# Patryk27/strolle

Measured on AMD Instinct MI355X. Metric: Mray/s (primary + shadow + GI rays traced per second, whole job), higher is better.
Workload: dtype f32

## Files before the change

include/strolle_hip.h:

```cpp
#ifndef STROLLE_HIP_H
#define STROLLE_HIP_H

#include <stddef.h>
#include <stdint.h>

#ifdef __cplusplus
extern "C" {
#endif

typedef struct StEngine StEngine;
typedef uint64_t StHandle;

enum StStatus {
    ST_OK = 0,
    ST_ERR_INVALID_ARGUMENT = 1,
    ST_ERR_NO_DEVICE = 2,
    ST_ERR_UNKNOWN_CAMERA = 3,
    ST_ERR_EMPTY_MESH = 4,
    ST_ERR_HIP = 5,
    ST_ERR_ATLAS_FULL = 6,
    ST_ERR_IO = 7,
    ST_ERR_PARSE = 8,
    ST_ERR_UNSUPPORTED = 9,
    ST_ERR_BVH_TOO_DEEP = 10,
// ... 303 lines not shown
    uint32_t alias_gi_history;
    uint32_t tile_map;
    uint32_t tile_map_denoise;
    int32_t side_priority;
    uint32_t staging;
    uint32_t double_buffer;
    uint32_t packed_base;
    uint32_t tick_timing;
    uint32_t anyhit_fast;
    uint32_t compact_bvh;
    uint32_t allow_deep_bvh;
    uint32_t device_bake;
    uint32_t wide_bvh;
    uint32_t wide_stack_entries;
    uint32_t primary_packets;
} StTuning;
int st_engine_get_tuning(StEngine* e, StTuning* out);
int st_engine_set_tuning(StEngine* e, const StTuning* tuning);

enum StArithmetic { ST_ARITH_FAST = 0, ST_ARITH_EXACT = 1 };
int st_engine_set_arithmetic(StEngine* e, int arithmetic);
int st_engine_get_arithmetic(StEngine* e, int* out);

enum StBufferId {
    ST_BUF_PRIM_GBUFFER_D0_A = 0, ST_BUF_PRIM_GBUFFER_D0_B = 1, ST_BUF_PRIM_GBUFFER_D1_A = 2, ST_BUF_PRIM_GBUFFER_D1_B = 3,
    ST_BUF_PRIM_SURFACE_MAP_A = 4, ST_BUF_PRIM_SURFACE_MAP_B = 5, ST_BUF_REPROJECTION_MAP = 6, ST_BUF_VELOCITY_MAP = 7,
    ST_BUF_DI_RESERVOIRS_0 = 8, ST_BUF_DI_RESERVOIRS_1 = 9, ST_BUF_DI_RESERVOIRS_2 = 10,
    ST_BUF_DI_DIFF_SAMPLES = 11, ST_BUF_DI_DIFF_PREV_COLORS = 12, ST_BUF_DI_DIFF_CURR_COLORS = 13,
    ST_BUF_DI_DIFF_MOMENTS_A = 14, ST_BUF_DI_DIFF_MOMENTS_B = 15, ST_BUF_DI_DIFF_STASH = 16, ST_BUF_DI_SPEC_SAMPLES = 17,
    ST_BUF_GI_D0 = 18, ST_BUF_GI_D1 = 19, ST_BUF_GI_D2 = 20,
    ST_BUF_GI_RESERVOIRS_0 = 21, ST_BUF_GI_RESERVOIRS_1 = 22, ST_BUF_GI_RESERVOIRS_2 = 23, ST_BUF_GI_RESERVOIRS_3 = 24,
    ST_BUF_GI_DIFF_SAMPLES = 25, ST_BUF_GI_DIFF_PREV_COLORS = 26, ST_BUF_GI_DIFF_CURR_COLORS = 27,
    ST_BUF_GI_DIFF_MOMENTS_A = 28, ST_BUF_GI_DIFF_MOMENTS_B = 29, ST_BUF_GI_DIFF_STASH = 30, ST_BUF_GI_SPEC_SAMPLES = 31,
// ... 75 lines not shown
```

rust/strolle-hip/src/ffi.rs:

```rust
#![allow(non_camel_case_types, dead_code)]
use std::ffi::c_void;
use std::os::raw::c_char;

#[repr(C)]
#[derive(Clone, Copy, Default)]
pub struct StMeshTriangle {
    pub positions: [[f32; 3]; 3],
    pub normals: [[f32; 3]; 3],
    pub uvs: [[f32; 2]; 3],
    pub tangents: [[f32; 4]; 3],
}

#[repr(C)]
#[derive(Clone, Copy, Default)]
pub struct StMaterial {
    pub base_color: [f32; 4],
    pub emissive: [f32; 4],
    pub perceptual_roughness: f32,
    pub metallic: f32,
    pub reflectance: f32,
    pub ior: f32,
    pub base_color_texture: u64,
    pub emissive_texture: u64,
    pub metallic_roughness_texture: u64,
// ... 28 lines not shown
    pub pos_x: u32,
    pub pos_y: u32,
    pub _pad: u32,
    pub transform: [f32; 16],
    pub projection: [f32; 16],
}

pub const ST_OK: i32 = 0;
pub const ST_FORMAT_RGBA32F: i32 = 0;
pub const ST_FORMAT_RGBA16F: i32 = 1;
pub const ST_FORMAT_RGBA8_UNORM_SRGB: i32 = 2;
pub const ST_FORMAT_BGRA8_UNORM_SRGB: i32 = 3;

pub const ST_ERR_BVH_TOO_DEEP: i32 = 10;
pub const ST_ERR_DIST: i32 = 11;

#[repr(C)]
#[derive(Clone, Copy, Default)]
pub struct StTuning {
    pub struct_size: u32,
    pub overlap: u32,
    pub fuse: u32,
    pub fuse_di_head: u32,
    pub fuse_spatial: u32,
    pub fuse_gi_sampling: u32,
    pub fuse_gi_validation: u32,
    pub fuse_gi_reprojection: u32,
    pub fuse_wavelet: u32,
    pub fuse_compose: u32,
    pub preview_both: u32,
// ... 4 lines not shown
    pub alias_gi_history: u32,
    pub tile_map: u32,
    pub tile_map_denoise: u32,
    pub side_priority: i32,
    pub staging: u32,
    pub double_buffer: u32,
    pub packed_base: u32,
    pub tick_timing: u32,
    pub anyhit_fast: u32,
    pub compact_bvh: u32,
    pub allow_deep_bvh: u32,
    pub device_bake: u32,
    pub wide_bvh: u32,
    pub wide_stack_entries: u32,
    pub primary_packets: u32,
}

#[repr(C)]
#[derive(Clone, Copy, PartialEq, Eq, Debug)]
pub struct StDistGrid {
    pub cols: u32,
    pub rows: u32,
    pub row_edge: [u32; 17],
    pub col_edge: [[u32; 17]; 16],
}

#[repr(C)]
#[derive(Clone, Copy, Default, PartialEq, Eq, Debug)]
pub struct StDistRect {
    pub x0: u32,
// ... 201 lines not shown
pub struct StDofDesc {
    pub struct_size: u32,
    pub flags: u32,
    pub samples: u32,
    pub focal_distance: f32,
    pub aperture_f_stops: f32,
    pub sensor_height: f32,
    pub max_radius: f32,
    pub focus_x: f32,
    pub focus_y: f32,
    pub _pad: u32,
}
extern "C" {
    pub fn st_camera_set_dof(e: *mut StEngine, camera: u64, desc: *const StDofDesc) -> i32;
    pub fn st_camera_get_dof(e: *mut StEngine, camera: u64, out: *mut StDofDesc, enabled: *mut i32) -> i32;
    pub fn st_dof_plan(desc: *const StDofDesc, width: u32, height: u32, samples: *mut u32, tiles_xy: *mut u32, taps_xyr: *mut f32) -> i32;
    pub fn st_dof_process(e: *mut StEngine, desc: *const StDofDesc, display: *const StDisplayDesc, projection: *const f32, color_device: *const c_void, depth_device: *const c_void, width: u32, height: u32, dst_device: *mut c_void, dst_format: i32, hip_stream: *mut c_void) -> i32;
}

pub type hipStream_t = *mut c_void;
extern "C" {
    pub fn hipMalloc(ptr: *mut *mut c_void, bytes: usize) -> i32;
    pub fn hipFree(ptr: *mut c_void) -> i32;
    pub fn hipHostMalloc(ptr: *mut *mut c_void, bytes: usize, flags: u32) -> i32;
    pub fn hipHostFree(ptr: *mut c_void) -> i32;
    pub fn hipStreamCreate(stream: *mut hipStream_t) -> i32;
    pub fn hipStreamDestroy(stream: hipStream_t) -> i32;
}
```

strolle_amd/api.py:

```python
from __future__ import annotations

import ctypes as C
import dataclasses
import enum
import math
import os
import sys
from typing import Optional, Sequence

import numpy as np

_HERE = os.path.dirname(os.path.abspath(__file__))
LIB_PATH = os.environ.get("STROLLE_HIP_LIB") or os.path.join(_HERE, "csrc", "libstrolle_hip.so")
if os.environ.get("STROLLE_HIP_LIB"):
    LIB_PATH = os.environ["STROLLE_HIP_LIB"]


class StMeshTriangle(C.Structure):
    _fields_ = [("positions", C.c_float * 9), ("normals", C.c_float * 9), ("uvs", C.c_float * 6), ("tangents", C.c_float * 12)]


class StSkinVertex(C.Structure):
    _fields_ = [("joints", C.c_uint16 * 4), ("weights", C.c_float * 4)]

# ... 44 lines not shown
    def describe(self):
        return {"cols": self.cols, "rows": self.rows, "row_edges": list(self.row_edge[:self.rows + 1]),
                "col_edges": [list(self.col_edge[k][:self.cols + 1]) for k in range(self.rows)]}


class StDistUniqueId(C.Structure):
    _fields_ = [("internal", C.c_char * 128)]


class StTuning(C.Structure):
    _fields_ = [(n, C.c_uint32) for n in ("struct_size", "overlap", "fuse", "fuse_di_head", "fuse_spatial", "fuse_gi_sampling", "fuse_gi_validation",
                                          "fuse_gi_reprojection", "fuse_wavelet", "fuse_compose", "preview_both", "variance_in_reproject",
                                          "lean_frame", "skip_scratch_stores", "di_head_on_main", "alias_gi_history", "tile_map", "tile_map_denoise")] + \
               [("side_priority", C.c_int32)] + \
               [(n, C.c_uint32) for n in ("staging", "double_buffer", "packed_base", "tick_timing", "anyhit_fast", "compact_bvh",
                                          "allow_deep_bvh", "device_bake", "wide_bvh", "wide_stack_entries", "primary_packets")]


PROFILE_MAX_KERNELS = 64


class StKernelProfile(C.Structure):
    _fields_ = [("name", C.c_char * 48), ("launches", C.c_uint32), ("total_ms", C.c_float), ("algorithmic_bytes", C.c_double), ("traversal_bytes", C.c_double)]


class StGltfOptions(C.Structure):
    _fields_ = [("first_handle", C.c_uint64), ("first_image_handle", C.c_uint64), ("override_mask", C.c_uint32), ("reflectance", C.c_float),
                ("perceptual_roughness", C.c_float), ("subdivide", C.c_uint32), ("light_radius", C.c_float), ("_pad", C.c_uint32)]


class StGltfSummary(C.Structure):
# ... 1183 lines not shown
```

strolle_amd/csrc/k_common.h:

```cpp
#pragma once
#include "st_device.h"
#include "st_passes.h"
#include "st_kernels.h"

namespace st {

constexpr int kBlockThreads = 256;
#ifdef ST_MIN_WAVES
#define ST_KERNEL_BOUNDS __launch_bounds__(kBlockThreads, ST_MIN_WAVES)
#else
#define ST_KERNEL_BOUNDS __launch_bounds__(kBlockThreads)
#endif
#define ST_STACK_LDS(SE, name) extern __shared__ __align__(16) unsigned char st_stack_lds_[]; SE* name = reinterpret_cast<SE*>(st_stack_lds_)
inline uint32_t stack_lds_bytes(const KArgs& a, size_t slot_bytes) { return a.stack_entries * (uint32_t)kBlockThreads * (uint32_t)slot_bytes; }

struct TileWindow { uint32_t tx0, tx1, ty0, ty1; };
__host__ __device__ inline TileWindow tile_window(const KArgs& a, bool half_x) {
    uint32_t tiles_x = (a.width + 7u) >> 3;
    if (half_x) tiles_x >>= 1;
    const uint32_t shift = half_x ? 4u : 3u, round = half_x ? 15u : 7u;
    TileWindow w;
    w.tx0 = a.col0 >> shift;
    w.tx1 = (a.col1 + round) >> shift; if (w.tx1 > tiles_x) w.tx1 = tiles_x;
    if (w.tx0 > w.tx1) w.tx0 = w.tx1;
// ... 2 lines not shown
    return w;
}
struct LaunchDims { uint32_t tiles_x, tile_x0, tile_y0, tile_y1, blocks; };
inline LaunchDims launch_dims(const KArgs& a, bool half_x) {
    const TileWindow w = tile_window(a, half_x);
    LaunchDims d;
    d.tiles_x = w.tx1 - w.tx0; d.tile_x0 = w.tx0;
    d.tile_y0 = w.ty0; d.tile_y1 = w.ty1;
    const uint32_t groups_x = (d.tiles_x + 3u) / 4u;
    d.blocks = groups_x * (d.tile_y1 - d.tile_y0);
    return d;
}

ST_D TileCoord resolve_tile(const KArgs& a, bool half_x) {
    const TileWindow w = tile_window(a, half_x);
    TileCoord tc = tile_for_thread(w.tx1 - w.tx0, w.ty1 - w.ty0, a.tile_map);
    tc.x += w.tx0; tc.y += w.ty0;
    return tc;
}
ST_D bool resolve_gid_of_block(const KArgs& a, bool half_x, uint32_t b, U2* gid) {
    const TileWindow w = tile_window(a, half_x);
    TileCoord tc = tile_for_block(b, w.tx1 - w.tx0, w.ty1 - w.ty0, a.tile_map);
    tc.x += w.tx0; tc.y += w.ty0;
    if (!tc.valid) return false;
    *gid = pixel_in_tile(tc);
    return true;
}
ST_D bool resolve_gid(const KArgs& a, bool half_x, U2* gid) {
    const TileCoord tc = resolve_tile(a, half_x);
    if (!tc.valid) return false;
    *gid = pixel_in_tile(tc);
    return true;
}
ST_D bool owns_pixel(const KArgs& a, U2 p) { return p.x < a.width && p.y < a.height && p.y >= a.row0 && p.y < a.row1 && p.x >= a.col0 && p.x < a.col1; }

constexpr uint32_t kStack16Texels = 4u * 65536u;
inline uint32_t stack16_limit(const KArgs& a) {
// ... 57 lines not shown
```

strolle_amd/csrc/k_denoise.hip:

```cpp
#include "k_common.h"

namespace st {
namespace ST_KNS {


struct f2 { float x, y; };
struct i2v { int x, y; };
ST_D f2 mk2(float x, float y) { f2 r; r.x = x; r.y = y; return r; }
ST_D f2 operator+(f2 a, f2 b) { return mk2(a.x + b.x, a.y + b.y); }
ST_D f2 operator-(f2 a, f2 b) { return mk2(a.x - b.x, a.y - b.y); }
ST_D f2 operator*(f2 a, f2 b) { return mk2(a.x * b.x, a.y * b.y); }
ST_D f2 operator*(f2 a, float b) { return mk2(a.x * b, a.y * b); }
ST_D f2 operator*(float a, f2 b) { return mk2(a * b.x, a * b.y); }
ST_D f2 operator+(f2 a, float b) { return mk2(a.x + b, a.y + b); }
ST_D f2 operator-(f2 a) { return mk2(-a.x, -a.y); }
ST_D f2 splat2(float x) { return mk2(x, x); }
ST_D f2 sqrt2(f2 x) { return mk2(fsqrt(x.x), fsqrt(x.y)); }
ST_D float div_by(float x, float d, float inv_d) {
#if ST_FAST_DEVICE
    return x * inv_d;
#else
    return x / d;
#endif
}
// ... 171 lines not shown
constexpr int kWvW = 32, kWvH = 16, kWvThreads = kWvW * kWvH;
struct WaveletBlock { int32_t x0, y0; bool valid; };
__host__ __device__ inline void wavelet_grid(const KArgs& a, uint32_t bw, uint32_t* bx0, uint32_t* groups_x, uint32_t* rows) {
    const uint32_t c1 = a.col1 < a.width ? a.col1 : a.width;
    *bx0 = a.col0 / bw;
    const uint32_t bx1 = (c1 + bw - 1u) / bw;
    *groups_x = bx1 > *bx0 ? bx1 - *bx0 : 0u;
    const uint32_t ty0 = a.row0 >> 3, ty1 = (a.row1 + 7u) >> 3;
    *rows = ((ty1 - ty0) * 8u + kWvH - 1u) / kWvH;
}
template <int BW = kWvW>
ST_D WaveletBlock wavelet_block(const KArgs& a) {
    uint32_t bx0, groups_x, rows;
    wavelet_grid(a, BW, &bx0, &groups_x, &rows);
    const uint32_t ty0 = a.row0 >> 3;
    const uint32_t n_blocks = groups_x * rows, b = blockIdx.x;
    uint32_t lin = b;
    if (a.tile_map == 0u) {
        const uint32_t q = n_blocks >> 3, r = n_blocks & 7u, xcd = b & 7u, k = b >> 3;
        lin = (xcd < r ? xcd * (q + 1u) : r * (q + 1u) + (xcd - r) * q) + k;
    } else if (a.tile_map == 2u) {
        const uint32_t chunk = groups_x * 2u * 8u, full = (n_blocks / chunk) * chunk;
        if (b < full) { const uint32_t c = b / chunk, i = b - c * chunk; lin = c * chunk + (i & 7u) * (groups_x * 2u) + (i >> 3); }
    }
    WaveletBlock w;
    const uint32_t gy = lin / groups_x, gx = lin - gy * groups_x;
    w.x0 = (int32_t)((bx0 + gx) * BW); w.y0 = (int32_t)(ty0 * 8u + gy * kWvH);
    w.valid = gy < rows;
    return w;
}
inline uint32_t wavelet_blocks(const KArgs& a, uint32_t block_w = kWvW) {
    uint32_t bx0, groups_x, rows;
    wavelet_grid(a, block_w, &bx0, &groups_x, &rows);
    return groups_x * rows;
}
ST_D bool wavelet_owns(const KArgs& a, int32_t px, int32_t py) { return px >= 0 && py >= 0 && owns_pixel(a, u2((uint32_t)px, (uint32_t)py)); }

void launch_denoise_variance(const KArgs& a, float4* di_out, float4* gi_out, hipStream_t s) { ST_LAUNCH(k_denoise_variance, false, s, a, di_out, gi_out); }

// ... 212 lines not shown
```

strolle_amd/csrc/st_abi.cpp:

```cpp
#include "st_engine.h"

using namespace st;
static Engine* E(StEngine* e) { return reinterpret_cast<Engine*>(e); }
#define ST_REQUIRE(cond, msg) do { if (!(cond)) return fail(ST_ERR_INVALID_ARGUMENT, msg); } while (0)

extern "C" {

const char* st_last_error(void) { return g_last_error.c_str(); }
#if __has_include("st_build_commit.inc")
#include "st_build_commit.inc"
#endif
#ifndef ST_BUILD_COMMIT
#define ST_BUILD_COMMIT "unknown"
#endif
const char* st_build_commit(void) { return ST_BUILD_COMMIT; }
extern "C" int st_internal_fail(int status, const char* message) { return fail(status, message ? message : ""); }

int st_engine_create(int device_ordinal, StEngine** out) {
    ST_REQUIRE(out, "out is NULL");
    std::unique_ptr<Engine> e(new Engine());
    if (device_ordinal >= 0) {
        int n = 0;
        if (hipGetDeviceCount(&n) != hipSuccess || n <= device_ordinal)
            return fail(ST_ERR_NO_DEVICE, "no HIP device with that ordinal (this library has no CPU rendering path)");
// ... 377 lines not shown
    return ST_OK;
}
int st_dof_plan(const StDofDesc* desc, uint32_t width, uint32_t height, uint32_t* samples, uint32_t tiles_xy[2], float taps_xyr[64 * 3]) {
    ST_REQUIRE(desc, "null desc");
    Engine::DofPlan plan;
    if (int rc = Engine::dof_plan(*desc, width, height, plan)) return rc;
    if (samples) *samples = plan.samples;
    if (tiles_xy) { tiles_xy[0] = plan.tiles_x; tiles_xy[1] = plan.tiles_y; }
    if (taps_xyr) for (uint32_t i = 0; i < kDofMaxSamples * 3u; i++) taps_xyr[i] = plan.taps[i];
    return ST_OK;
}
int st_dof_process(StEngine* e, const StDofDesc* desc, const StDisplayDesc* display, const float projection[16], const void* color, const void* depth,
                   uint32_t width, uint32_t height, void* dst, int dst_format, void* stream) {
    ST_REQUIRE(e, "null engine");
    return E(e)->dof_process(desc, display, projection, color, depth, width, height, dst, dst_format, static_cast<hipStream_t>(stream));
}

int st_debug_set_bloom_tail(StEngine* e, int lds_bytes, uint32_t* in_force) {
    ST_REQUIRE(e, "null engine");
    ST_REQUIRE(lds_bytes >= -1, "lds_bytes is -1 (what the device grants), 0 (no fused tail) or a byte count");
    E(e)->bloom_tail_wanted = lds_bytes;
    if (in_force) *in_force = E(e)->bloom_tail_bytes();
    return ST_OK;
}

int st_tick(StEngine* e, void* stream) { ST_REQUIRE(e, "null engine"); return E(e)->tick(static_cast<hipStream_t>(stream)); }
int st_render_camera(StEngine* e, StHandle h, void* out, void* stream) {
    ST_REQUIRE(e, "null engine");
    auto it = E(e)->cameras.find(h);
    if (it == E(e)->cameras.end()) return fail(ST_ERR_UNKNOWN_CAMERA, "camera does not exist");
// ... 367 lines not shown
```

strolle_amd/csrc/st_aov.cpp:

```cpp
#include "st_engine.h"

namespace st {

int Engine::render_aovs(const CameraState& c, const StAovTargets& t, hipStream_t stream) {
    KArgs a;
    if (int rc = query_begin(stream, a, true)) return rc;
    a.cam = c.has_shown ? c.shown : c.curr; a.prev_cam = c.has_shown ? c.shown_prev : c.prev;
    a.width = c.has_shown ? c.shown_width : c.desc.width; a.height = c.has_shown ? c.shown_height : c.desc.height;
    a.row0 = c.row0; a.row1 = c.row1; a.col0 = c.col0; a.col1 = c.col1;
    a.tile_map = tuning.tile_map;
    L.launch_aov(a, static_cast<float*>(t.planes[ST_AOV_DEPTH]), static_cast<float4*>(t.planes[ST_AOV_NORMAL]), static_cast<float4*>(t.planes[ST_AOV_ALBEDO]),
                 static_cast<float2*>(t.planes[ST_AOV_MOTION]), static_cast<uint64_t*>(t.planes[ST_AOV_INSTANCE]), static_cast<uint32_t*>(t.planes[ST_AOV_TRIANGLE]),
                 static_cast<const uint4*>(sets[live].instance_table.ptr), t.planes[ST_AOV_MOTION] ? deform.deform_posed() : nullptr, stream);
    ST_HIP(hipGetLastError());
    return reader_end(stream, false, t.planes[ST_AOV_MOTION] != nullptr);
}

}
```

strolle_amd/csrc/st_device.h:

```cpp
#pragma once
#include "st_types.h"

namespace st {

#define ST_D __device__ __forceinline__

struct TileCoord { uint32_t x, y; bool valid; };
ST_D TileCoord tile_for_block(uint32_t b, uint32_t tiles_x, uint32_t tiles_y, uint32_t map_mode) {
    const uint32_t groups_x = (tiles_x + 3u) >> 2;
    const uint32_t n_blocks = groups_x * tiles_y;
    uint32_t lin = b;
    if (map_mode == 0u) {
        const uint32_t q = n_blocks >> 3, r = n_blocks & 7u;
        const uint32_t xcd = b & 7u, k = b >> 3;
        lin = (xcd < r ? xcd * (q + 1u) : r * (q + 1u) + (xcd - r) * q) + k;
    } else if (map_mode == 2u) {
        const uint32_t chunk = groups_x * 4u * 8u;
        const uint32_t full = (n_blocks / chunk) * chunk;
        if (b < full) {
            const uint32_t c = b / chunk, i = b - c * chunk;
            const uint32_t xcd = i & 7u, k = i >> 3;
            lin = c * chunk + xcd * (groups_x * 4u) + k;
        }
    }
    const uint32_t wave = threadIdx.x >> 6;
    TileCoord t;
    t.y = lin / groups_x;
    t.x = (lin - t.y * groups_x) * 4u + wave;
    t.valid = b < n_blocks && t.x < tiles_x && t.y < tiles_y;
    return t;
}
ST_D TileCoord tile_for_thread(uint32_t tiles_x, uint32_t tiles_y, uint32_t map_mode) { return tile_for_block(blockIdx.x, tiles_x, tiles_y, map_mode); }
ST_D U2 pixel_in_tile(TileCoord t) {
    const uint32_t lane = threadIdx.x & 63u;
    return u2(t.x * 8u + (lane & 7u), t.y * 8u + (lane >> 3));
}
template <class SE>
ST_D SE* lane_stack(const KArgs& a, SE* lds) { return lds + (threadIdx.x >> 6) * (a.stack_entries * 64u) + (threadIdx.x & 63u); }

ST_D void count_rays_n(const KArgs& a, uint32_t rays , unsigned long long used_memory) {
    unsigned long long* line = a.ray_counter + (blockIdx.x & (kCounterLines - 1u)) * 8u;
    if (rays & 1u) atomicAdd(line, 1ull);
    if (rays & 2u) atomicAdd(line, 2ull);
    if (a.count_bytes) atomicAdd(line + 1, used_memory);
}
ST_D void count_rays_many(const KArgs& a, uint32_t rays, unsigned long long used_memory) {
    unsigned long long* line = a.ray_counter + (blockIdx.x & (kCounterLines - 1u)) * 8u;
// ... 813 lines not shown
```

strolle_amd/csrc/st_engine.cpp:

```cpp
#include "st_engine.h"

namespace st {

thread_local std::string g_last_error;
thread_local LaunchEvents g_launch_events;

StTuning default_tuning() {
    StTuning t{};
    t.struct_size = sizeof(StTuning);
    t.overlap = t.fuse = t.fuse_di_head = t.fuse_spatial = t.fuse_gi_sampling = t.fuse_gi_validation = t.fuse_gi_reprojection = 1u;
    t.fuse_wavelet = t.fuse_compose = t.preview_both = t.variance_in_reproject = t.lean_frame = 1u;
    t.skip_scratch_stores = t.di_head_on_main = t.alias_gi_history = 1u;
    t.tile_map = 1u; t.tile_map_denoise = 2u; t.side_priority = 0;
    t.staging = t.double_buffer = t.packed_base = 1u; t.tick_timing = 0u;
    t.anyhit_fast = 1u; t.compact_bvh = 1u; t.wide_bvh = 1u; t.primary_packets = 1u;
    t.allow_deep_bvh = 0u; t.device_bake = 1u;
    return t;
}
static void tuning_from_environment(StTuning& t) {
    struct Clear { const char* name; uint32_t StTuning::*field; };
    static const Clear clears[] = {
        {"ST_NO_OVERLAP", &StTuning::overlap}, {"ST_NO_FUSE", &StTuning::fuse}, {"ST_NO_FUSE_DI_HEAD", &StTuning::fuse_di_head},
        {"ST_NO_FUSE_SPATIAL", &StTuning::fuse_spatial}, {"ST_NO_FUSE_GI_SAMPLING", &StTuning::fuse_gi_sampling},
        {"ST_NO_FUSE_GI_VALIDATION", &StTuning::fuse_gi_validation}, {"ST_NO_FUSE_GI_REPROJECTION", &StTuning::fuse_gi_reprojection},
        {"ST_NO_FUSE_WAVELET", &StTuning::fuse_wavelet}, {"ST_NO_FUSE_COMPOSE", &StTuning::fuse_compose}, {"ST_NO_PREVIEW_BOTH", &StTuning::preview_both},
        {"ST_NO_VARIANCE_IN_REPROJECT", &StTuning::variance_in_reproject},
        {"ST_KEEP_ALL_PLANES", &StTuning::lean_frame}, {"ST_KEEP_SCRATCH", &StTuning::skip_scratch_stores}, {"ST_NO_GI_ALIAS", &StTuning::alias_gi_history},
        {"ST_NO_STAGING", &StTuning::staging}, {"ST_NO_DOUBLE_BUFFER", &StTuning::double_buffer}, {"ST_NO_PACKED_BASE", &StTuning::packed_base},
        {"ST_NO_ANYHIT_FAST", &StTuning::anyhit_fast}, {"ST_NO_COMPACT_BVH", &StTuning::compact_bvh}, {"ST_NO_WIDE_BVH", &StTuning::wide_bvh}, {"ST_NO_PRIMARY_PACKETS", &StTuning::primary_packets},
    };
    for (const Clear& c : clears) if (const char* v = getenv(c.name)) { if (atoi(v) != 0) t.*c.field = 0u; else if (t.*c.field == 0u) t.*c.field = 1u; }
    struct Value { const char* name; uint32_t StTuning::*field; };
    static const Value values[] = {
        {"ST_DI_HEAD_ON_MAIN", &StTuning::di_head_on_main}, {"ST_TILE_MAP_DENOISE", &StTuning::tile_map_denoise}, {"ST_TICK_TIMING", &StTuning::tick_timing},
        {"ST_ALLOW_DEEP_BVH", &StTuning::allow_deep_bvh}, {"ST_DEVICE_BAKE", &StTuning::device_bake},
    };
    if (const char* v = getenv("ST_TILE_MAP")) t.tile_map = t.tile_map_denoise = (uint32_t)atoi(v);
    for (const Value& c : values) if (const char* v = getenv(c.name)) t.*c.field = (uint32_t)atoi(v);
    if (const char* v = getenv("ST_SIDE_PRIORITY")) t.side_priority = atoi(v);
}

Engine::Engine() {
    GpuLight sun{};
    sun.d0 = make_float4(0, 0, 0, 25.0f); sun.d1 = make_float4(0, 0, 0, INFINITY); sun.d2 = make_float4(b2f(1u), 0, 0, 0);
    light_buffer.push_back(sun);
    light_slot[-1] = 0;
    blue_noise.assign(256 * 256 * 4, 0);
    reset_profile_totals();
    tuning = default_tuning();
    tuning_from_environment(tuning);
    staging.enabled = tuning.staging != 0u;
    if (const char* x = getenv("ST_BLOOM_TAIL_BYTES")) bloom_tail_wanted = atoi(x);
    if (const char* x = getenv("ST_EXP")) exp_flags = (uint32_t)strtoul(x, nullptr, 0);
    if (const char* ex = getenv("ST_EXACT")) if (atoi(ex) != 0) { arithmetic = ST_ARITH_EXACT; L = launchers_exact(); }
}
int Engine::set_tuning(const StTuning& t) {
    if (t.struct_size != sizeof(StTuning)) return fail(ST_ERR_INVALID_ARGUMENT, "StTuning::struct_size does not match this library");
    if (t.tile_map > 2u || t.tile_map_denoise > 2u) return fail(ST_ERR_INVALID_ARGUMENT, "tile_map is 0, 1 or 2");
    if (t.wide_stack_entries != 0u && (t.wide_stack_entries < 8u || t.wide_stack_entries > 56u)) return fail(ST_ERR_INVALID_ARGUMENT, "wide_stack_entries is 0 (default) or 8 ... 56");
    if (t.wide_stack_entries != tuning.wide_stack_entries) wide_stack_rearmed = 0u;
    tuning = t;
    staging.enabled = tuning.staging != 0u;
    return ST_OK;
}
void Engine::note_walk_overflow() {
    const bool lane = walk_flags_host[0] != 0u, packet = walk_flags_host[1] != 0u;
    walk_flags_host[0] = 0u; walk_flags_host[1] = 0u;
    if (!lane && !packet) return;
    walk_overflows++; walk_overflow_unreported = true;
    if (packet) packets_overflowed = true;
    if (lane) {
        const uint32_t now = wide_stack_entries_now();
        wide_stack_rearmed = now < 32u ? 32u : (now < 48u ? 48u : 56u);
// ... 18 lines not shown
```

strolle_amd/csrc/st_render.cpp:

```cpp
#include "st_engine.h"

namespace st {

void Engine::release_camera(CameraState& c) {
    c.slab.release(); c.counters.release(); c.tile_mask.release();
    c.side_stream.reset();
    for (Event* e : {&c.ev_di_head, &c.ev_gi_done, &c.ev_prim_ok, &c.ev_frame_done, &c.ev_setup}) e->reset();
    c.have_prev_frame_events = false;
    c.join_present(); c.present_stream.reset();
    for (auto& p : c.present) p = CameraState::PresentSlot();
}

int Engine::present_copy(CameraState& c, const void* src, void* dst, size_t bytes, hipStream_t stream) {
    if (!has_device) return fail(ST_ERR_NO_DEVICE, "present copy on a host-only engine");
    ST_HIP(hipSetDevice(device));
    if (!c.present_stream) ST_HIP(hipStreamCreateWithFlags(&c.present_stream.h, hipStreamNonBlocking));
    CameraState::PresentSlot* slot = nullptr;
    for (auto& p : c.present) if (p.dst == dst) slot = &p;
    if (!slot) { slot = &c.present[c.present_next & 1u]; c.present_next++; }
    if (slot->pending) ST_HIP(hipEventSynchronize(slot->ev_done.h));
    slot->src = src; slot->dst = dst;
    if (int rc = slot->ev_src.record(stream)) return rc;
    if (int rc = slot->ev_src.wait(c.present_stream)) return rc;
    ST_HIP(hipMemcpyAsync(dst, src, bytes, hipMemcpyDeviceToHost, c.present_stream));
// ... 202 lines not shown
        a.sm = P(alt ? ST_BUF_PRIM_SURFACE_MAP_B : ST_BUF_PRIM_SURFACE_MAP_A); a.psm = P(alt ? ST_BUF_PRIM_SURFACE_MAP_A : ST_BUF_PRIM_SURFACE_MAP_B);
        a.sn = P(ST_BUF_COUNT + (alt ? 1 : 0)); a.psn = P(ST_BUF_COUNT + (alt ? 0 : 1));
        a.reprojection = P(ST_BUF_REPROJECTION_MAP); a.velocity = P(ST_BUF_VELOCITY_MAP);
        for (int i = 0; i < 3; i++) a.di_res[i] = P(ST_BUF_DI_RESERVOIRS_0 + i);
        a.di_diff_samples = P(ST_BUF_DI_DIFF_SAMPLES); a.di_diff_prev_colors = P(ST_BUF_DI_DIFF_PREV_COLORS); a.di_diff_curr_colors = P(ST_BUF_DI_DIFF_CURR_COLORS);
        a.di_diff_moments = P(alt ? ST_BUF_DI_DIFF_MOMENTS_B : ST_BUF_DI_DIFF_MOMENTS_A); a.di_diff_prev_moments = P(alt ? ST_BUF_DI_DIFF_MOMENTS_A : ST_BUF_DI_DIFF_MOMENTS_B);
        a.di_diff_stash = P(ST_BUF_DI_DIFF_STASH); a.di_spec_samples = P(ST_BUF_DI_SPEC_SAMPLES);
        a.gi_d0 = P(ST_BUF_GI_D0); a.gi_d1 = P(ST_BUF_GI_D1); a.gi_d2 = P(ST_BUF_GI_D2);
        for (int i = 0; i < 4; i++) a.gi_res[i] = P(ST_BUF_GI_RESERVOIRS_0 + i);
        a.gi_diff_samples = P(ST_BUF_GI_DIFF_SAMPLES); a.gi_diff_prev_colors = P(ST_BUF_GI_DIFF_PREV_COLORS); a.gi_diff_curr_colors = P(ST_BUF_GI_DIFF_CURR_COLORS);
        a.gi_diff_moments = P(alt ? ST_BUF_GI_DIFF_MOMENTS_B : ST_BUF_GI_DIFF_MOMENTS_A); a.gi_diff_prev_moments = P(alt ? ST_BUF_GI_DIFF_MOMENTS_A : ST_BUF_GI_DIFF_MOMENTS_B);
        a.gi_diff_stash = P(ST_BUF_GI_DIFF_STASH); a.gi_spec_samples = P(ST_BUF_GI_SPEC_SAMPLES);
        a.ref_hits = P(ST_BUF_REF_HITS); a.ref_rays = P(ST_BUF_REF_RAYS); a.ref_colors = P(ST_BUF_REF_COLORS);
        a.dbg_used_memory = reinterpret_cast<uint32_t*>(P(ST_BUF_DBG_USED_MEMORY));
        a.width = c.desc.width; a.height = c.desc.height; a.row0 = c.row0; a.row1 = c.row1; a.col0 = c.col0; a.col1 = c.col1;
        a.frame = c.frame; a.tile_map = e.tuning.tile_map;
        return ST_OK;
    }
    int decide_switches() {
        e.last_launches.clear();
        if (mode != ST_MODE_BVH_HEATMAP && mode != ST_MODE_REFERENCE) {
            a.tile_mask = c.tile_mask.as<unsigned long long>();
            a.gi_late_mask = a.tile_mask ? a.tile_mask + c.tile_mask_tiles() : nullptr;
        }
        const StTuning& t = e.tuning; const bool fast = e.arithmetic == ST_ARITH_FAST;
        s.needs_di = mode == ST_MODE_IMAGE || mode == ST_MODE_DI_DIFFUSE || mode == ST_MODE_DI_SPECULAR;
        s.needs_gi = mode == ST_MODE_IMAGE || mode == ST_MODE_GI_DIFFUSE || mode == ST_MODE_GI_SPECULAR;
        s.denoise = c.desc.denoise != 0u; s.any_objects = !e.instances.empty();
        s.tracing = c.frame % 6u < 4u; s.gi_source = (s.tracing && c.frame % 2u == 1u) ? 1u : 0u;
        s.whole_graph = e.pass_mask == ~0ull;
        s.gi_runs = s.needs_gi && s.any_objects;
// ... 114 lines not shown
            a.gi_mid_src = (a.lean & kLeanGiMid) ? gi_preview_src() : nullptr;
            run(KS_GI_PREVIEW_LATE, group, [&] { e.L.launch_gi_preview_resolve(a, pseed, 1u, a.gi_res[3], gi_source, dn, cur); });
            a.gi_preview_late = 0u; a.gi_mid_src = nullptr;
            if (dn) gi_reprojected = true;
        } else if (e.tuning.fuse) {
            if (dn) { run(KS_GI_PREVIEW_RESOLVE_REPROJECT, ST_PASS_GI_PREVIEW_1 | ST_PASS_GI_RESOLVING | ST_PASS_DENOISE_REPROJECT_GI, [&] { e.L.launch_gi_preview_resolve(a, pseed, 1u, a.gi_res[3], gi_source, true, cur); }); gi_reprojected = true; }
            else run(KS_GI_PREVIEW_RESOLVE, ST_PASS_GI_PREVIEW_1 | ST_PASS_GI_RESOLVING, [&] { e.L.launch_gi_preview_resolve(a, pseed, 1u, a.gi_res[3], gi_source, false, cur); });
        } else {
            run(KS_GI_PREVIEW, ST_PASS_GI_PREVIEW_1, [&] { e.L.launch_gi_preview(a, pseed, 1u, a.gi_res[3], a.gi_res[0], cur); });
            run(KS_GI_RESOLVING, ST_PASS_GI_RESOLVING, [&] { e.L.launch_gi_resolving(a, gi_source, cur); });
        }
        if (s.swap_gi_history) { std::swap(c.plane[ST_BUF_GI_RESERVOIRS_0], c.plane[ST_BUF_GI_RESERVOIRS_1]); c.gi_aliased = true; }
    }
    void denoise() {
        if (!s.denoise) return;
        struct MapScope { KArgs& a; uint32_t saved; MapScope(KArgs& a_, uint32_t m) : a(a_), saved(a_.tile_map) { a.tile_map = m; } ~MapScope() { a.tile_map = saved; } } map_scope(a, e.tuning.tile_map_denoise);
        if (!di_reprojected) run(KS_DENOISE_REPROJECT, ST_PASS_DENOISE_REPROJECT_DI, [&] { e.L.launch_denoise_reproject(a, a.di_diff_prev_colors, a.di_diff_prev_moments, a.di_diff_samples, a.di_diff_curr_colors, a.di_diff_moments, cur); });
        if (!gi_reprojected) run(KS_DENOISE_REPROJECT, ST_PASS_DENOISE_REPROJECT_GI, [&] { e.L.launch_denoise_reproject(a, a.gi_diff_prev_colors, a.gi_diff_prev_moments, a.gi_diff_samples, a.gi_diff_curr_colors, a.gi_diff_moments, cur); });
        float4* di[3] = {a.di_diff_stash, a.di_diff_prev_colors, a.di_diff_curr_colors};
        float4* gi[3] = {a.gi_diff_stash, a.gi_diff_prev_colors, a.gi_diff_curr_colors};
        const int in_ix[5] = {0, 1, 0, 2, 0}, out_ix[5] = {1, 0, 2, 0, 2};
        uint32_t first = 0;
        if (e.tuning.fuse && e.tuning.fuse_wavelet) {
            const uint64_t group = ST_PASS_DENOISE_VARIANCE | ST_PASS_DENOISE_WAVELET_0 | ((uint64_t)ST_PASS_DENOISE_WAVELET_0 << 1);
            float4* tmp_di = a.variance_in_reproject ? a.di_diff_curr_colors : c.plane[ST_BUF_COUNT + 2];
            float4* tmp_gi = a.variance_in_reproject ? a.gi_diff_curr_colors : c.plane[ST_BUF_COUNT + 3];
            run(KS_DENOISE_VARIANCE, group, [&] { e.L.launch_denoise_variance(a, tmp_di, tmp_gi, cur); });
            run(KS_DENOISE_WAVELET_12, group, [&] { e.L.launch_denoise_wavelet_12(a, 1.0f, 2.0f, tmp_di, di[1], di[0], tmp_gi, gi[1], gi[0], cur); });
            first = 2;
        } else run(KS_DENOISE_VARIANCE, ST_PASS_DENOISE_VARIANCE, [&] { e.L.launch_denoise_variance(a, a.di_diff_stash, a.gi_diff_stash, cur); });
        for (uint32_t nth = first; nth < 5; nth++) {
            if (nth == 4u && s.compose_in_wavelet) {
                Engine::present_guard(c, out, cur); e.dist_guard(c.handle, out, cur);
                run(KS_DENOISE_WAVELET_COMPOSE, ((uint64_t)ST_PASS_DENOISE_WAVELET_0 << nth) | ST_PASS_COMPOSITION, [&] {
                    e.L.launch_denoise_wavelet_compose(a, 1u << nth, (float)(1u + nth), di[in_ix[nth]], di[out_ix[nth]], gi[in_ix[nth]], gi[out_ix[nth]], mode, route.comp_out, route.comp_format, a.lean == 0u, route.comp_disp, cur); });
                composed = true;
                continue;
            }
            run(KS_DENOISE_WAVELET, (uint64_t)ST_PASS_DENOISE_WAVELET_0 << nth, [&] { e.L.launch_denoise_wavelet(a, 1u << nth, (float)(1u + nth), di[in_ix[nth]], di[out_ix[nth]], gi[in_ix[nth]], gi[out_ix[nth]], cur); });
        }
    }
    void blur_pack() {
        if (!route.mblur) return;
        run(blur.step[0].slot, ST_PASS_POST, [&] { e.launch_mblur_step(blur.step[0], cur); }, blur.step[0].bytes);
    }
    void dof_pack() {
// ... 109 lines not shown
```

strolle_amd/csrc/st_types.h:

```cpp
#pragma once
#include "st_math.h"

namespace st {

struct GpuCamera {
    M4 projection_view;
    M4 ndc_to_world;
    float4 origin;
    float4 screen;
};
static_assert(sizeof(GpuCamera) == 160, "Camera uniform is 160 B");

struct GpuMaterial {
    float4 base_color, base_color_texture, emissive, emissive_texture;
    float roughness, metallic, reflectance, ior;
    float4 metallic_roughness_texture, normal_map_texture;
};
static_assert(sizeof(GpuMaterial) == 112, "Material is 112 B");

struct GpuLight { float4 d0, d1, d2, d3, prev_d0, prev_d1, prev_d2; };
static_assert(sizeof(GpuLight) == 112, "Light is 112 B");

struct HostTriangle { float4 d0, d1, d2, d3, d4, d5, d6, d7, d8; };
static_assert(sizeof(HostTriangle) == 144, "Triangle is 144 B");
// ... 56 lines not shown
    uint32_t width, height, tiles_x, tiles_y, frame, samples, jitter, format, raw;
    float half_shutter, max_radius, depth_softness;
    DisplayArgs display;
};

constexpr uint32_t kDofTile = 32u, kDofMaxSamples = 64u;
struct DofArgs {
    const void* depth; const float4* color;
    float2* packed; float* tile_max; float* tile_n; void* dst;
    uint32_t width, height, tiles_x, tiles_y, frame, samples, format, raw, planar, autofocus, focus_px, focus_py;
    float p0, p5, p8, p9, focal_length , k , focal_distance, max_radius;
    DisplayArgs display;
    float taps[kDofMaxSamples * 3u];
};

struct KArgs {
    GpuCamera cam, prev_cam;
    const float4* bvh; const float4* tri_attr;
    const float4* instance_xforms;
    const GpuMaterial* materials; const GpuLight* lights;
    const GpuLight* lights_lds;
    const uint32_t* material_base_packed;
    const uchar4* atlas; const uchar4* blue_noise;
    const float* byte_luts;
    const float4* transmittance_lut; const float4* sky_lut;
    uint32_t bvh_len, n_lights_buf, light_count, atlas_w, atlas_h;
    uint32_t stack_entries;
    unsigned long long* tile_mask; uint32_t variance_in_reproject;
    unsigned long long* gi_late_mask; uint32_t gi_preview_late;
    uint32_t skip_dead_scratch;
// ... 26 lines not shown
    float4* gi_res[4];
    float4 *gi_diff_samples, *gi_diff_prev_colors, *gi_diff_curr_colors, *gi_diff_moments, *gi_diff_stash, *gi_spec_samples;
    const float4* gi_diff_prev_moments;
    float4 *ref_hits, *ref_rays, *ref_colors;
    uint32_t* dbg_used_memory;
    unsigned long long* ray_counter;
    uint32_t width, height, row0, row1;
    uint32_t col0, col1;
    uint32_t frame;
    uint32_t tile_map;
    const float4* env_map;
    const EnvCell* env_table;
    uint32_t env_w, env_h, env_gw, env_gh;
    float env_intensity, env_cos_yaw, env_sin_yaw;
    uint32_t env_uniform;
};

}
```

Before: 9889.

## Add region-banded XCD block ordering for wide-stride a-trous passes

Adds a block-to-tile mapping that splits the grid into eight column bands and assigns each XCD its own band, rotating the band by row group. Blocks on one XCD then touch a contiguous screen region, aiming to keep large-stride a-trous wavelet reads within that XCD's L2. It is enabled by default only for a-trous passes with stride 4 or more (bit 0); ReSTIR and the near SVGF passes keep the old mapping unless turned on. It also adds a host-side debug function that checks the mapping is a bijection.

```diff
diff --git a/include/strolle_hip.h b/include/strolle_hip.h
--- a/include/strolle_hip.h
+++ b/include/strolle_hip.h
@@ -341,9 +341,21 @@
     uint32_t wide_bvh;
     uint32_t wide_stack_entries;
     uint32_t primary_packets;
+    uint32_t tile_regions;
 } StTuning;
 int st_engine_get_tuning(StEngine* e, StTuning* out);
 int st_engine_set_tuning(StEngine* e, const StTuning* tuning);
+typedef struct StBlockOrderReport {
+    uint32_t blocks;
+    uint32_t bijection;
+    uint32_t outside;
+    uint32_t same_as_mode;
+    uint32_t bands_distinct;
+    uint32_t x, y;
+    uint32_t band_x, band_y;
+} StBlockOrderReport;
+int st_debug_block_order(uint32_t groups_x, uint32_t rows, uint32_t geometry, uint32_t family, uint32_t mode, uint32_t tile_regions, uint32_t b,
+                         StBlockOrderReport* out);
 
 enum StArithmetic { ST_ARITH_FAST = 0, ST_ARITH_EXACT = 1 };
 int st_engine_set_arithmetic(StEngine* e, int arithmetic);
diff --git a/rust/strolle-hip/src/ffi.rs b/rust/strolle-hip/src/ffi.rs
--- a/rust/strolle-hip/src/ffi.rs
+++ b/rust/strolle-hip/src/ffi.rs
@@ -66,6 +66,20 @@
 
 pub const ST_ERR_BVH_TOO_DEEP: i32 = 10;
 pub const ST_ERR_DIST: i32 = 11;
+
+#[repr(C)]
+#[derive(Clone, Copy, Default)]
+pub struct StBlockOrderReport {
+    pub blocks: u32,
+    pub bijection: u32,
+    pub outside: u32,
+    pub same_as_mode: u32,
+    pub bands_distinct: u32,
+    pub x: u32,
+    pub y: u32,
+    pub band_x: u32,
+    pub band_y: u32,
+}
 
 #[repr(C)]
 #[derive(Clone, Copy, Default)]
@@ -100,6 +114,7 @@
     pub wide_bvh: u32,
     pub wide_stack_entries: u32,
     pub primary_packets: u32,
+    pub tile_regions: u32,
 }
 
 #[repr(C)]
@@ -331,6 +346,7 @@
 extern "C" {
     pub fn st_camera_set_dof(e: *mut StEngine, camera: u64, desc: *const StDofDesc) -> i32;
     pub fn st_camera_get_dof(e: *mut StEngine, camera: u64, out: *mut StDofDesc, enabled: *mut i32) -> i32;
+    pub fn st_debug_block_order(groups_x: u32, rows: u32, geometry: u32, family: u32, mode: u32, tile_regions: u32, b: u32, out: *mut StBlockOrderReport) -> i32;
     pub fn st_dof_plan(desc: *const StDofDesc, width: u32, height: u32, samples: *mut u32, tiles_xy: *mut u32, taps_xyr: *mut f32) -> i32;
     pub fn st_dof_process(e: *mut StEngine, desc: *const StDofDesc, display: *const StDisplayDesc, projection: *const f32, color_device: *const c_void, depth_device: *const c_void, width: u32, height: u32, dst_device: *mut c_void, dst_format: i32, hip_stream: *mut c_void) -> i32;
 }
diff --git a/strolle_amd/api.py b/strolle_amd/api.py
--- a/strolle_amd/api.py
+++ b/strolle_amd/api.py
@@ -82,7 +82,23 @@
                                           "lean_frame", "skip_scratch_stores", "di_head_on_main", "alias_gi_history", "tile_map", "tile_map_denoise")] + \
                [("side_priority", C.c_int32)] + \
                [(n, C.c_uint32) for n in ("staging", "double_buffer", "packed_base", "tick_timing", "anyhit_fast", "compact_bvh",
-                                          "allow_deep_bvh", "device_bake", "wide_bvh", "wide_stack_entries", "primary_packets")]
+                                          "allow_deep_bvh", "device_bake", "wide_bvh", "wide_stack_entries", "primary_packets", "tile_regions")]
+
+
+class StBlockOrderReport(C.Structure):
+    _fields_ = [(n, C.c_uint32) for n in ("blocks", "bijection", "outside", "same_as_mode", "bands_distinct", "x", "y", "band_x", "band_y")]
+
+
+def block_order(groups_x: int, rows: int, geometry: int, family: int, mode: int, tile_regions: int, b: int = 0) -> StBlockOrderReport:
+    lib = load_library()
+    lib.st_debug_block_order.restype = C.c_int
+    lib.st_debug_block_order.argtypes = [C.c_uint32] * 7 + [C.POINTER(StBlockOrderReport)]
+    out = StBlockOrderReport()
+    rc = lib.st_debug_block_order(groups_x, rows, geometry, family, mode, tile_regions, b, C.byref(out))
+    if rc != 0:
+        lib.st_last_error.restype = C.c_char_p
+        raise StrolleError(f"{_STATUS.get(rc, 'error')} (status {rc}): {lib.st_last_error().decode(errors='replace')}")
+    return out
 
 
 PROFILE_MAX_KERNELS = 64
diff --git a/strolle_amd/csrc/k_common.h b/strolle_amd/csrc/k_common.h
--- a/strolle_amd/csrc/k_common.h
+++ b/strolle_amd/csrc/k_common.h
@@ -40,13 +40,13 @@
 
 ST_D TileCoord resolve_tile(const KArgs& a, bool half_x) {
     const TileWindow w = tile_window(a, half_x);
-    TileCoord tc = tile_for_thread(w.tx1 - w.tx0, w.ty1 - w.ty0, a.tile_map);
+    TileCoord tc = tile_for_thread(w.tx1 - w.tx0, w.ty1 - w.ty0, a.tile_map, a.tile_regions);
     tc.x += w.tx0; tc.y += w.ty0;
     return tc;
 }
 ST_D bool resolve_gid_of_block(const KArgs& a, bool half_x, uint32_t b, U2* gid) {
     const TileWindow w = tile_window(a, half_x);
-    TileCoord tc = tile_for_block(b, w.tx1 - w.tx0, w.ty1 - w.ty0, a.tile_map);
+    TileCoord tc = tile_for_block(b, w.tx1 - w.tx0, w.ty1 - w.ty0, a.tile_map, a.tile_regions);
     tc.x += w.tx0; tc.y += w.ty0;
     if (!tc.valid) return false;
     *gid = pixel_in_tile(tc);
diff --git a/strolle_amd/csrc/k_denoise.hip b/strolle_amd/csrc/k_denoise.hip
--- a/strolle_amd/csrc/k_denoise.hip
+++ b/strolle_amd/csrc/k_denoise.hip
@@ -209,15 +209,7 @@
     uint32_t bx0, groups_x, rows;
     wavelet_grid(a, BW, &bx0, &groups_x, &rows);
     const uint32_t ty0 = a.row0 >> 3;
-    const uint32_t n_blocks = groups_x * rows, b = blockIdx.x;
-    uint32_t lin = b;
-    if (a.tile_map == 0u) {
-        const uint32_t q = n_blocks >> 3, r = n_blocks & 7u, xcd = b & 7u, k = b >> 3;
-        lin = (xcd < r ? xcd * (q + 1u) : r * (q + 1u) + (xcd - r) * q) + k;
-    } else if (a.tile_map == 2u) {
-        const uint32_t chunk = groups_x * 2u * 8u, full = (n_blocks / chunk) * chunk;
-        if (b < full) { const uint32_t c = b / chunk, i = b - c * chunk; lin = c * chunk + (i & 7u) * (groups_x * 2u) + (i >> 3); }
-    }
+    const uint32_t lin = block_order(blockIdx.x, groups_x, rows, a.tile_map, kWaveletChunkRows, a.tile_regions);
     WaveletBlock w;
     const uint32_t gy = lin / groups_x, gx = lin - gy * groups_x;
     w.x0 = (int32_t)((bx0 + gx) * BW); w.y0 = (int32_t)(ty0 * 8u + gy * kWvH);
diff --git a/strolle_amd/csrc/st_abi.cpp b/strolle_amd/csrc/st_abi.cpp
--- a/strolle_amd/csrc/st_abi.cpp
+++ b/strolle_amd/csrc/st_abi.cpp
@@ -415,6 +415,41 @@
                    uint32_t width, uint32_t height, void* dst, int dst_format, void* stream) {
     ST_REQUIRE(e, "null engine");
     return E(e)->dof_process(desc, display, projection, color, depth, width, height, dst, dst_format, static_cast<hipStream_t>(stream));
+}
+
+struct BlockCoord { uint32_t x, y; };
+int st_debug_block_order(uint32_t groups_x, uint32_t rows, uint32_t geometry, uint32_t family, uint32_t mode, uint32_t tile_regions, uint32_t b, StBlockOrderReport* out) {
+    ST_REQUIRE(out, "null report");
+    ST_REQUIRE(groups_x >= 1u && rows >= 1u && groups_x <= 4096u && rows <= 4096u, "a grid is 1 ... 4096 blocks each way");
+    ST_REQUIRE(geometry <= 1u && family <= 2u && mode <= 2u && tile_regions <= 7u, "geometry is 0 or 1, family 0, 1 or 2, mode 0, 1 or 2, tile_regions 0 ... 7");
+    const uint32_t chunk_rows = geometry == 0u ? kTileChunkRows : kWaveletChunkRows;
+    const uint32_t regions = tile_regions & (1u << family);
+    const uint32_t n = groups_x * rows, core = regions ? block_regions_core(groups_x, rows) : 0u, cw = groups_x >> 3;
+    auto band_y_of = [&](uint32_t y) { uint32_t c = 0u; while (c < 7u && (c + 1u) * rows / 8u <= y) c++; return c; };
+    std::vector<uint8_t> seen(n, 0);
+    uint8_t owner[8][8], column[8][8];
+    memset(owner, 0, sizeof(owner)); memset(column, 0, sizeof(column));
+    StBlockOrderReport r{};
+    r.blocks = n; r.outside = n - core; r.bijection = 1u; r.same_as_mode = 1u; r.bands_distinct = core ? 1u : 0u;
+    for (uint32_t i = 0; i < n; i++) {
+        const uint32_t lin = block_order(i, groups_x, rows, mode, chunk_rows, regions);
+        const BlockCoord at = {lin % groups_x, lin / groups_x};
+        if (lin >= n || seen[lin]++) r.bijection = 0u;
+        if (lin != block_order(i, groups_x, rows, mode, chunk_rows, 0u)) r.same_as_mode = 0u;
+        if (i < core && at.x < cw * 8u && at.y < rows) {
+            const uint32_t by = band_y_of(at.y), bx = at.x / cw, xcd = i & 7u;
+            if ((owner[by][bx] && owner[by][bx] != xcd + 1u) || (column[by][xcd] && column[by][xcd] != bx + 1u)) r.bands_distinct = 0u;
+            owner[by][bx] = (uint8_t)(xcd + 1u); column[by][xcd] = (uint8_t)(bx + 1u);
+        } else if (i < core) r.bands_distinct = 0u;
+    }
+    for (uint32_t c = 0; core && c < 8u; c++) for (uint32_t j = 0; j < 8u; j++) if (!owner[c][j] || !column[c][j]) r.bands_distinct = 0u;
+    const uint32_t lin = block_order(b, groups_x, rows, mode, chunk_rows, regions);
+    const BlockCoord at = {lin % groups_x, lin / groups_x};
+    r.x = at.x; r.y = at.y;
+    const bool inside = b < core && at.x < cw * 8u && at.y < rows;
+    r.band_x = inside ? at.x / cw : 0xffffffffu; r.band_y = inside ? band_y_of(at.y) : 0xffffffffu;
+    *out = r;
+    return ST_OK;
 }
 
 int st_debug_set_bloom_tail(StEngine* e, int lds_bytes, uint32_t* in_force) {
diff --git a/strolle_amd/csrc/st_aov.cpp b/strolle_amd/csrc/st_aov.cpp
--- a/strolle_amd/csrc/st_aov.cpp
+++ b/strolle_amd/csrc/st_aov.cpp
@@ -8,7 +8,7 @@
     a.cam = c.has_shown ? c.shown : c.curr; a.prev_cam = c.has_shown ? c.shown_prev : c.prev;
     a.width = c.has_shown ? c.shown_width : c.desc.width; a.height = c.has_shown ? c.shown_height : c.desc.height;
     a.row0 = c.row0; a.row1 = c.row1; a.col0 = c.col0; a.col1 = c.col1;
-    a.tile_map = tuning.tile_map;
+    a.tile_map = tuning.tile_map; a.tile_regions = tuning.tile_regions & kRegionsRestir;
     L.launch_aov(a, static_cast<float*>(t.planes[ST_AOV_DEPTH]), static_cast<float4*>(t.planes[ST_AOV_NORMAL]), static_cast<float4*>(t.planes[ST_AOV_ALBEDO]),
                  static_cast<float2*>(t.planes[ST_AOV_MOTION]), static_cast<uint64_t*>(t.planes[ST_AOV_INSTANCE]), static_cast<uint32_t*>(t.planes[ST_AOV_TRIANGLE]),
                  static_cast<const uint4*>(sets[live].instance_table.ptr), t.planes[ST_AOV_MOTION] ? deform.deform_posed() : nullptr, stream);
diff --git a/strolle_amd/csrc/st_device.h b/strolle_amd/csrc/st_device.h
--- a/strolle_amd/csrc/st_device.h
+++ b/strolle_amd/csrc/st_device.h
@@ -6,23 +6,10 @@
 #define ST_D __device__ __forceinline__
 
 struct TileCoord { uint32_t x, y; bool valid; };
-ST_D TileCoord tile_for_block(uint32_t b, uint32_t tiles_x, uint32_t tiles_y, uint32_t map_mode) {
+ST_D TileCoord tile_for_block(uint32_t b, uint32_t tiles_x, uint32_t tiles_y, uint32_t map_mode, uint32_t regions) {
     const uint32_t groups_x = (tiles_x + 3u) >> 2;
     const uint32_t n_blocks = groups_x * tiles_y;
-    uint32_t lin = b;
-    if (map_mode == 0u) {
-        const uint32_t q = n_blocks >> 3, r = n_blocks & 7u;
-        const uint32_t xcd = b & 7u, k = b >> 3;
-        lin = (xcd < r ? xcd * (q + 1u) : r * (q + 1u) + (xcd - r) * q) + k;
-    } else if (map_mode == 2u) {
-        const uint32_t chunk = groups_x * 4u * 8u;
-        const uint32_t full = (n_blocks / chunk) * chunk;
-        if (b < full) {
-            const uint32_t c = b / chunk, i = b - c * chunk;
-            const uint32_t xcd = i & 7u, k = i >> 3;
-            lin = c * chunk + xcd * (groups_x * 4u) + k;
-        }
-    }
+    const uint32_t lin = block_order(b, groups_x, tiles_y, map_mode, kTileChunkRows, regions);
     const uint32_t wave = threadIdx.x >> 6;
     TileCoord t;
     t.y = lin / groups_x;
@@ -30,7 +17,7 @@
     t.valid = b < n_blocks && t.x < tiles_x && t.y < tiles_y;
     return t;
 }
-ST_D TileCoord tile_for_thread(uint32_t tiles_x, uint32_t tiles_y, uint32_t map_mode) { return tile_for_block(blockIdx.x, tiles_x, tiles_y, map_mode); }
+ST_D TileCoord tile_for_thread(uint32_t tiles_x, uint32_t tiles_y, uint32_t map_mode, uint32_t regions) { return tile_for_block(blockIdx.x, tiles_x, tiles_y, map_mode, regions); }
 ST_D U2 pixel_in_tile(TileCoord t) {
     const uint32_t lane = threadIdx.x & 63u;
     return u2(t.x * 8u + (lane & 7u), t.y * 8u + (lane >> 3));
diff --git a/strolle_amd/csrc/st_engine.cpp b/strolle_amd/csrc/st_engine.cpp
--- a/strolle_amd/csrc/st_engine.cpp
+++ b/strolle_amd/csrc/st_engine.cpp
@@ -15,6 +15,7 @@
     t.staging = t.double_buffer = t.packed_base = 1u; t.tick_timing = 0u;
     t.anyhit_fast = 1u; t.compact_bvh = 1u; t.wide_bvh = 1u; t.primary_packets = 1u;
     t.allow_deep_bvh = 0u; t.device_bake = 1u;
+    t.tile_regions = 1u;
     return t;
 }
 static void tuning_from_environment(StTuning& t) {
@@ -33,7 +34,7 @@
     struct Value { const char* name; uint32_t StTuning::*field; };
     static const Value values[] = {
         {"ST_DI_HEAD_ON_MAIN", &StTuning::di_head_on_main}, {"ST_TILE_MAP_DENOISE", &StTuning::tile_map_denoise}, {"ST_TICK_TIMING", &StTuning::tick_timing},
-        {"ST_ALLOW_DEEP_BVH", &StTuning::allow_deep_bvh}, {"ST_DEVICE_BAKE", &StTuning::device_bake},
+        {"ST_ALLOW_DEEP_BVH", &StTuning::allow_deep_bvh}, {"ST_DEVICE_BAKE", &StTuning::device_bake}, {"ST_TILE_REGIONS", &StTuning::tile_regions},
     };
     if (const char* v = getenv("ST_TILE_MAP")) t.tile_map = t.tile_map_denoise = (uint32_t)atoi(v);
     for (const Value& c : values) if (const char* v = getenv(c.name)) t.*c.field = (uint32_t)atoi(v);
@@ -57,6 +58,7 @@
 int Engine::set_tuning(const StTuning& t) {
     if (t.struct_size != sizeof(StTuning)) return fail(ST_ERR_INVALID_ARGUMENT, "StTuning::struct_size does not match this library");
     if (t.tile_map > 2u || t.tile_map_denoise > 2u) return fail(ST_ERR_INVALID_ARGUMENT, "tile_map is 0, 1 or 2");
+    if (t.tile_regions > 7u) return fail(ST_ERR_INVALID_ARGUMENT, "tile_regions is 0 ... 7 (bit 0: the a-trous passes of stride 4 and more, bit 1: the ReSTIR passes, bit 2: the other SVGF passes)");
     if (t.wide_stack_entries != 0u && (t.wide_stack_entries < 8u || t.wide_stack_entries > 56u)) return fail(ST_ERR_INVALID_ARGUMENT, "wide_stack_entries is 0 (default) or 8 ... 56");
     if (t.wide_stack_entries != tuning.wide_stack_entries) wide_stack_rearmed = 0u;
     tuning = t;
diff --git a/strolle_amd/csrc/st_render.cpp b/strolle_amd/csrc/st_render.cpp
--- a/strolle_amd/csrc/st_render.cpp
+++ b/strolle_amd/csrc/st_render.cpp
@@ -240,7 +240,7 @@
         a.ref_hits = P(ST_BUF_REF_HITS); a.ref_rays = P(ST_BUF_REF_RAYS); a.ref_colors = P(ST_BUF_REF_COLORS);
         a.dbg_used_memory = reinterpret_cast<uint32_t*>(P(ST_BUF_DBG_USED_MEMORY));
         a.width = c.desc.width; a.height = c.desc.height; a.row0 = c.row0; a.row1 = c.row1; a.col0 = c.col0; a.col1 = c.col1;
-        a.frame = c.frame; a.tile_map = e.tuning.tile_map;
+        a.frame = c.frame; a.tile_map = e.tuning.tile_map; a.tile_regions = e.tuning.tile_regions & kRegionsRestir;
         return ST_OK;
     }
     int decide_switches() {
@@ -385,7 +385,11 @@
     }
     void denoise() {
         if (!s.denoise) return;
-        struct MapScope { KArgs& a; uint32_t saved; MapScope(KArgs& a_, uint32_t m) : a(a_), saved(a_.tile_map) { a.tile_map = m; } ~MapScope() { a.tile_map = saved; } } map_scope(a, e.tuning.tile_map_denoise);
+        struct MapScope {
+            KArgs& a; uint32_t saved, saved_regions;
+            MapScope(KArgs& a_, uint32_t m, uint32_t regions) : a(a_), saved(a_.tile_map), saved_regions(a_.tile_regions) { a.tile_map = m; a.tile_regions = regions; }
+            ~MapScope() { a.tile_map = saved; a.tile_regions = saved_regions; }
+        } map_scope(a, e.tuning.tile_map_denoise, e.tuning.tile_regions & kRegionsSvgfNear);
         if (!di_reprojected) run(KS_DENOISE_REPROJECT, ST_PASS_DENOISE_REPROJECT_DI, [&] { e.L.launch_denoise_reproject(a, a.di_diff_prev_colors, a.di_diff_prev_moments, a.di_diff_samples, a.di_diff_curr_colors, a.di_diff_moments, cur); });
         if (!gi_reprojected) run(KS_DENOISE_REPROJECT, ST_PASS_DENOISE_REPROJECT_GI, [&] { e.L.launch_denoise_reproject(a, a.gi_diff_prev_colors, a.gi_diff_prev_moments, a.gi_diff_samples, a.gi_diff_curr_colors, a.gi_diff_moments, cur); });
         float4* di[3] = {a.di_diff_stash, a.di_diff_prev_colors, a.di_diff_curr_colors};
@@ -401,6 +405,7 @@
             first = 2;
         } else run(KS_DENOISE_VARIANCE, ST_PASS_DENOISE_VARIANCE, [&] { e.L.launch_denoise_variance(a, a.di_diff_stash, a.gi_diff_stash, cur); });
         for (uint32_t nth = first; nth < 5; nth++) {
+            a.tile_regions = e.tuning.tile_regions & ((1u << nth) >= kRegionsFarStride ? kRegionsAtrousFar : kRegionsSvgfNear);
             if (nth == 4u && s.compose_in_wavelet) {
                 Engine::present_guard(c, out, cur); e.dist_guard(c.handle, out, cur);
                 run(KS_DENOISE_WAVELET_COMPOSE, ((uint64_t)ST_PASS_DENOISE_WAVELET_0 << nth) | ST_PASS_COMPOSITION, [&] {
diff --git a/strolle_amd/csrc/st_types.h b/strolle_amd/csrc/st_types.h
--- a/strolle_amd/csrc/st_types.h
+++ b/strolle_amd/csrc/st_types.h
@@ -94,6 +94,45 @@
     float taps[kDofMaxSamples * 3u];
 };
 
+__host__ __device__ inline uint32_t block_regions_core(uint32_t groups_x, uint32_t rows) {
+    return groups_x >= 8u && rows >= 8u ? (groups_x >> 3) * 8u * rows : 0u;
+}
+__host__ __device__ inline uint32_t block_order_rows(uint32_t b, uint32_t groups_x, uint32_t n_blocks, uint32_t mode, uint32_t chunk_rows) {
+    uint32_t lin = b;
+    if (mode == 0u) {
+        const uint32_t q = n_blocks >> 3, r = n_blocks & 7u;
+        const uint32_t xcd = b & 7u, k = b >> 3;
+        lin = (xcd < r ? xcd * (q + 1u) : r * (q + 1u) + (xcd - r) * q) + k;
+    } else if (mode == 2u) {
+        const uint32_t chunk = groups_x * chunk_rows * 8u;
+        const uint32_t full = (n_blocks / chunk) * chunk;
+        if (b < full) {
+            const uint32_t c = b / chunk, i = b - c * chunk;
+            const uint32_t xcd = i & 7u, k = i >> 3;
+            lin = c * chunk + xcd * (groups_x * chunk_rows) + k;
+        }
+    }
+    return lin;
+}
+__host__ __device__ inline uint32_t block_order_regions(uint32_t b, uint32_t groups_x, uint32_t rows, uint32_t chunk_rows) {
+    const uint32_t cw = groups_x >> 3, core = cw * 8u * rows;
+    if (b < core) {
+        const uint32_t xcd = b & 7u, k = b >> 3, y = k / cw;
+        const uint32_t band = ((y + 1u) * 8u - 1u) / rows;
+        return y * groups_x + ((xcd + band) & 7u) * cw + (k - y * cw);
+    }
+    const uint32_t rest_x = groups_x & 7u;
+    const uint32_t lin = block_order_rows(b - core, rest_x, rest_x * rows, 2u, chunk_rows), y = lin / rest_x;
+    return y * groups_x + cw * 8u + (lin - y * rest_x);
+}
+__host__ __device__ inline uint32_t block_order(uint32_t b, uint32_t groups_x, uint32_t rows, uint32_t mode, uint32_t chunk_rows, uint32_t regions) {
+    const uint32_t n_blocks = groups_x * rows;
+    if (regions != 0u && groups_x >= 8u && rows >= 8u && b < n_blocks) return block_order_regions(b, groups_x, rows, chunk_rows);
+    return block_order_rows(b, groups_x, n_blocks, mode, chunk_rows);
+}
+constexpr uint32_t kRegionsAtrousFar = 1u, kRegionsRestir = 2u, kRegionsSvgfNear = 4u, kRegionsFarStride = 4u;
+constexpr uint32_t kTileChunkRows = 4u, kWaveletChunkRows = 2u;
+
 struct KArgs {
     GpuCamera cam, prev_cam;
     const float4* bvh; const float4* tri_attr;
@@ -150,6 +189,7 @@
     uint32_t env_w, env_h, env_gw, env_gh;
     float env_intensity, env_cos_yaw, env_sin_yaw;
     uint32_t env_uniform;
+    uint32_t tile_regions;
 };
 
 }
```

New measurement: 9881 (median of 2 runs). No clear change (-0.1%).
